# HKUST-Aerial-Robotics/D2SLAM

Measured on AMD Instinct MI355X. Metric: frames/sec SuperPoint+NetVLAD+match, 640x480 stereo, higher is better.
Workload: dtype f32

## Files before the change

d2slam_amd/csrc/conv1x1.hip:

```cpp
#include "conv_common.h"

namespace d2fe {

namespace {
constexpr int C1_CIN = 256, C1_C8 = C1_CIN / 8, C1_RING = 8;
}

__global__ __launch_bounds__(256, 2) void conv1x1_256_65_kernel(ConvArgs a, long npix) {
  extern __shared__ __attribute__((aligned(16))) float wsm[];
  const int tid = threadIdx.x, lane = tid & 63, wave = tid >> 6, hh = lane >> 5;
  const float* wp = reinterpret_cast<const float*>(a.wpack);
  for (int i = tid; i < 2 * C1_C8 * 64; i += 256)
    reinterpret_cast<f32x4*>(wsm)[i] = reinterpret_cast<const f32x4*>(wp)[i];
  float* wdl = wsm + 2 * C1_C8 * 256;
  if (tid < C1_C8 * 8) {
    const int g = tid >> 3, h = (tid >> 2) & 1, q = tid & 3;
    wdl[tid] = wp[((size_t)2 * C1_C8 + g) * 256 + h * 128 + q];
  }
  const float bias0 = a.bias[lane & 31], bias1 = a.bias[32 + (lane & 31)], biasd = a.bias[64];
  __syncthreads();

  const long n_mt = (npix + 31) / 32;
  const int ics = a.in_cstride, ocs = a.out_cstride;
  for (long mt = (long)blockIdx.x * 4 + wave; mt < n_mt; mt += (long)gridDim.x * 4) {
    const long p = mt * 32 + (lane & 31);
    const bool valid = p < npix;
    const float* row = a.in + (size_t)(valid ? p : 0) * ics + a.in_coff;
    f32x16 acc0, acc1;
#pragma unroll
    for (int r = 0; r < 16; ++r) { acc0[r] = bias0; acc1[r] = bias1; }
    float d = biasd;
    f32x4 xa[C1_RING][2];
#pragma unroll
    for (int g = 0; g < C1_RING; ++g) {
      xa[g][0] = *reinterpret_cast<const f32x4*>(row + g * 8);
      xa[g][1] = *reinterpret_cast<const f32x4*>(row + g * 8 + 4);
    }
#pragma unroll 1
    for (int g0 = 0; g0 < C1_C8; g0 += C1_RING) {
#pragma unroll
      for (int gg = 0; gg < C1_RING; ++gg) {
        const int g = g0 + gg;
        const f32x4 x0 = xa[gg][0], x1 = xa[gg][1];
        if (g + C1_RING < C1_C8) {
          xa[gg][0] = *reinterpret_cast<const f32x4*>(row + (g + C1_RING) * 8);
          xa[gg][1] = *reinterpret_cast<const f32x4*>(row + (g + C1_RING) * 8 + 4);
        }
        const f32x4 b0 = reinterpret_cast<const f32x4*>(wsm)[(0 * C1_C8 + g) * 64 + lane];
        const f32x4 b1 = reinterpret_cast<const f32x4*>(wsm)[(1 * C1_C8 + g) * 64 + lane];
        const float a0 = hh ? x0[1] : x0[0], a1 = hh ? x0[3] : x0[2], a2 = hh ? x1[1] : x1[0], a3 = hh ? x1[3] : x1[2];
        acc0 = __builtin_amdgcn_mfma_f32_32x32x2f32(a0, b0[0], acc0, 0, 0, 0);
        acc1 = __builtin_amdgcn_mfma_f32_32x32x2f32(a0, b1[0], acc1, 0, 0, 0);
        acc0 = __builtin_amdgcn_mfma_f32_32x32x2f32(a1, b0[1], acc0, 0, 0, 0);
        acc1 = __builtin_amdgcn_mfma_f32_32x32x2f32(a1, b1[1], acc1, 0, 0, 0);
        acc0 = __builtin_amdgcn_mfma_f32_32x32x2f32(a2, b0[2], acc0, 0, 0, 0);
        acc1 = __builtin_amdgcn_mfma_f32_32x32x2f32(a2, b1[2], acc1, 0, 0, 0);
        acc0 = __builtin_amdgcn_mfma_f32_32x32x2f32(a3, b0[3], acc0, 0, 0, 0);
        acc1 = __builtin_amdgcn_mfma_f32_32x32x2f32(a3, b1[3], acc1, 0, 0, 0);
        const f32x4 we = reinterpret_cast<const f32x4*>(wdl)[g * 2], wo = reinterpret_cast<const f32x4*>(wdl)[g * 2 + 1];
        d = __builtin_fmaf(x0[0], we[0], d);   d = __builtin_fmaf(x0[1], wo[0], d);
        d = __builtin_fmaf(x0[2], we[1], d);   d = __builtin_fmaf(x0[3], wo[1], d);
        d = __builtin_fmaf(x1[0], we[2], d);   d = __builtin_fmaf(x1[1], wo[2], d);
        d = __builtin_fmaf(x1[2], we[3], d);   d = __builtin_fmaf(x1[3], wo[3], d);
      }
    }
    float* out = a.out + a.out_coff;
#pragma unroll
    for (int r = 0; r < 16; ++r) {
      const long pp = mt * 32 + (r & 3) + 8 * (r >> 2) + 4 * hh;
      if (pp < npix) {
        out[(size_t)pp * ocs + (lane & 31)] = acc0[r];
        out[(size_t)pp * ocs + 32 + (lane & 31)] = acc1[r];
      }
    }
    if (valid && hh == 0) out[(size_t)p * ocs + 64] = d;
  }
}

hipError_t launch_conv1x1_256_65(const ConvArgs& a, hipStream_t s) {
  const long hw = (long)a.H * a.W;
  if (a.cout_real != 65 || a.in_img_stride != hw * a.in_cstride || a.out_img_stride != hw * a.out_cstride || a.out_cstride < 65 ||
      (a.in_cstride & 3) || (a.in_coff & 3) || a.in_coff + 256 > a.in_cstride)
    return hipErrorNotSupported;
  const int ncu = a.ncu > 0 ? a.ncu : 256;
  const long npix = hw * a.n_img;
  const long n_wg = (npix + 127) / 128;
  const int grid = (int)(n_wg < 2 * ncu ? n_wg : 2 * ncu);
  constexpr size_t lds = (size_t)(2 * C1_C8 * 256 + C1_C8 * 8) * sizeof(float);
  hipError_t e = hipFuncSetAttribute(reinterpret_cast<const void*>(conv1x1_256_65_kernel), hipFuncAttributeMaxDynamicSharedMemorySize, (int)lds);
  if (e != hipSuccess) return e;
  hipLaunchKernelGGL(conv1x1_256_65_kernel, dim3(grid), dim3(256), lds, s, a, npix);
  return hipGetLastError();
}

}
```

d2slam_amd/csrc/kernels.h:

```cpp
#pragma once
#include <hip/hip_runtime.h>
#include <stdint.h>

#ifdef D2FE_DEVTOOLS
#include <cstdlib>
static inline int d2fe_dev_env(const char* name, int dflt) { const char* e = getenv(name); return e ? atoi(e) : dflt; }
#define D2FE_ABL(a, bits) ((a).ablate & (bits))
#define D2FE_STAMP(buf, wg, i) do { if ((buf) && threadIdx.x == 0) (buf)[(size_t)(wg) * 16 + (i)] = wall_clock64(); } while (0)
#else
static inline int d2fe_dev_env(const char*, int dflt) { return dflt; }
#define D2FE_ABL(a, bits) (0)
#define D2FE_STAMP(buf, wg, i) do {} while (0)
#endif

#ifdef D2FE_DEVTOOLS
#include "../../include/d2fe_debug.h"
namespace d2fe { void regime_note(int regime); void regime_set(int regime, long long value); }
#define D2FE_REGIME(r) ::d2fe::regime_note(r)
#define D2FE_REGIME_SET(r, v) ::d2fe::regime_set(r, v)
#else
#define D2FE_REGIME(r) do {} while (0)
#define D2FE_REGIME_SET(r, v) do {} while (0)
#endif

namespace d2fe {

__host__ __device__ inline bool wino_claims_items(const int* work_ctr, int total, int grid) { return work_ctr != nullptr && total >= 48 * grid; }

struct ConvArgs {
  const float* in;  int in_cstride;  int in_coff;
  float* out;       int out_cstride; int out_coff;
  int cout_real;
  const void* wpack;
  const float* bias;
  int H, W;
  int n_img;
  long in_img_stride;
  long out_img_stride;
  const uint8_t* img; int img_stride; long img_istride; const float* w1a; const float* b1a;
  const float* zeros;
  int tag;
  int ablate;
  int* work_ctr = nullptr;
  int ncu = 0;
};

enum ConvShape {
  CONV_64_T8x32 = 0,
  CONV_128_T4x32,
  CONV_128_T4x16,
  CONV_256_1x1_T4x16,
  CONV1B_FUSED,
};

hipError_t launch_conv(ConvShape shape, int precision, bool pool, bool relu, int cout_pad, const ConvArgs& a,
                       hipStream_t s);

hipError_t launch_conv1x1_256_65(const ConvArgs& a, hipStream_t s);

hipError_t launch_conv_pc(ConvShape shape, int precision, bool pool, bool relu, int cout_pad, const ConvArgs& a, hipStream_t s);

hipError_t launch_conv_wino(int cin, bool pool, bool relu, int cout_pad, const ConvArgs& a, hipStream_t s);
hipError_t launch_conv_wino_fused1b(int cout_pad, const ConvArgs& a, hipStream_t s);
size_t packed_weight_floats_wino(int cout_pad, int cin);
void pack_weights_wino(const float* w , int cout, int cin, int cout_pad, float* dst);

hipError_t launch_conv1a(const uint8_t* img, int stride, long img_stride_bytes, int H, int W, int n,
                         const float* w9x64 , const float* bias, float* out, hipStream_t s);

size_t packed_weight_floats_f32(int cout_pad, int cin, int ks);
void pack_weights_f32(const float* w , int cout, int cin, int ks, int cout_pad, float* dst);
size_t packed_weight_halfs_f16x2(int cout_pad, int cin, int ks);
void pack_weights_f16x2(const float* w, int cout, int cin, int ks, int cout_pad, uint16_t* dst);

hipError_t launch_softmax_cand(const float* logits, int lstride, int Hc, int Wc, int n_img, float thr, int border,
                               float* semi, unsigned long long* cand, int* cand_count, long cand_cap, bool zero_counts, hipStream_t s);
hipError_t launch_select_b(const unsigned long long* cand, const int* cand_count, long cand_cap, int n_img, int W,
                           int max_kp, int cap, int always_sort, const float* semi, int H, float thr, int border, float* kps_xy,
                           float* scores, int32_t* kps_idx, int32_t* n_out, hipStream_t s);
hipError_t launch_sample_b(const float* desc_raw, int dstride, int dcoff, int Hc, int Wc, int n_img, const float* kps_xy,
                           const int32_t* n_kp, int cap, const int32_t* slotmap, int max_slots, float* desc_out, hipStream_t s);
hipError_t launch_desc_head_sparse(const float* kps_xy, const int32_t* n_kp, int cap, int Hc, int Wc, int n_img, const float* x,
                                   int x_cstride, long x_img_stride, const void* w_da, const float* b_da, const void* w_db,
                                   const float* b_db, uint8_t* flags, int32_t* slotmap, int32_t* cells, int32_t* count,
                                   int max_slots, float* out, float* mid, int mid_imgs, int img_w, int img_h, hipStream_t s);

hipError_t launch_nms2_a(const float* semi, int H, int W, int n_img, float thr, int dist, float* aconf, int* clist,
                         unsigned long long* cand, int* cand_count, long cand_cap, int* ncand, hipStream_t s);
hipError_t launch_nms2_wrap_fix(const int* clist, const int* ncand, int H, int W, int n_img, float* kps_xy, int32_t* kps_idx,
                                const int32_t* n_kp, int cap, hipStream_t s);
hipError_t launch_sample_a(const float* desc_raw, int dstride, int dcoff, int Hc, int Wc, int img_w, int img_h, int n_img,
                           const float* kps_xy, const int32_t* n_kp, int cap, const float* comp_t, const float* mean,
                           int pca_dims, float* samp, int scap, float* cn, const int32_t* slotmap, int max_slots, float* desc_out,
                           hipStream_t s);

hipError_t launch_nv_conv0(const uint8_t* img, int stride_b, long img_stride, int H, int W, int Ho, int Wo, int cstride,
                           int cout, int act, const float* w, const float* b, float* out, int n, hipStream_t s);
hipError_t launch_nv_dw(const float* in, int H, int W, int C, int Ho, int Wo, int cstride, int act, const float* w, const float* b,
                        float* out, int n, hipStream_t s);
hipError_t launch_nv_pw(const float* in, long P, int Cin, int Cout, int CoutPad, int act, const float* w, const float* b,
                        const float* res, float* out, hipStream_t s);
hipError_t launch_nv_vlad(const float* x, int slabs, long slab_stride, int np, int D, int K, const float* aw, const float* aw_pack,
                          const float* ab, const float* cen, float* part, float* out, int n, hipStream_t s);
void pack_nv_assign(const float* aw , int K, int D, float* dst);
size_t nv_vlad_part_floats(int np, int D, int K);
hipError_t launch_nv_pca(const float* x, int nfeat, const float* comp, const float* mean, int m, float* y, int n, hipStream_t s);

struct NvBlockArgs {
  const float* in;
  int in_slabs; long in_slab_stride;
  const uint8_t* img; int img_stride; long img_istride; int H0, W0;
  int c0_stride, c0_pt, c0_pl, act0; const float* w0;
  float* out; long out_slab_stride;
  const float* res; int res_slabs; long res_slab_stride;
  int H, W, Cin, Chid, Cout, stride, Ho, Wo, pt, pl;
  int co0, Cv;
  long P;
  int th, tw;
  unsigned inv_iw, inv_tw;
  int cpg;
  int gmerge;
  const float* we;
  const float* wp;
  const float* bp;
  int act_e, act_d, act_p;
  int ncu;
  int tpw;
  int nbuf;
  unsigned long long* stamps;
};
bool nv_block_supported(int cin, int chid, int cout, int stride, bool expand, int mode);
int nv_block_ntiles(int cout);
hipError_t launch_nv_block(const NvBlockArgs& a, bool expand, int mode, int n, int groups, hipStream_t s);
void pack_nv_expand(const float* w , const float* b, int chid, int cin, float* dst);
size_t pack_nv_expand_floats(int chid, int cin);
void pack_nv_dwproj(const float* wd , const float* bd, const float* wp , int cout, int chid, int nt, float* dst);
size_t pack_nv_dwproj_floats(int chid, int nt);
void pack_nv_proj_t(const float* wp, int cout, int chid, int nt, float* dst);
void pack_nv_dwproj_x(const float* wd, const float* bd, const float* wp, int cout, int chid, int nt, float* dst);
void pack_nv_expand_tail(const float* w, const float* b, int chid, int cin, float* dst);
bool nv_tail_supported(int cin, int cout);
hipError_t launch_nv_tail(const NvBlockArgs& a, int groups, hipStream_t s);
bool nv_xblock_supported(int cin, int chid, int cout, int stride);
void nv_xblock_tile(int Ho, int Wo, int stride, int* th, int* tw);
size_t pack_nv_expand_perm_floats(int chid, int cin);
void pack_nv_expand_perm(const float* w, const float* b, int chid, int cin, float* dst);
hipError_t launch_nv_xblock(const NvBlockArgs& a, int n, int groups, hipStream_t s);
bool nv_pblock_supported(int cin, int chid, int cout, int stride);
void nv_pblock_tile(int Ho, int Wo, int* th, int* tw, int c0_stride = 0);
size_t pack_nv_expand_pair_floats(int chid, int cin);
void pack_nv_expand_pair(const float* w, const float* b, int chid, int cin, float* dst);
size_t pack_nv_dwproj_pair_floats(int chid, int nt);
void pack_nv_dwproj_pair(const float* wd, const float* bd, const float* wp, int cout, int chid, int nt, float* dst, int co0 = 0);
int nv_pblock_ntiles(int cout);
int nv_pblock_halves(int cout);
int nv_pblock_half_cout(int cout, int half);
bool nv_pblock_single_input(int cin);
hipError_t launch_nv_pblock(const NvBlockArgs& a, int n, int groups, hipStream_t s);
bool nv_fpair_supported(int c0_cout, int c0_stride, int dw_stride, int cout);
hipError_t launch_nv_fpair(const NvBlockArgs& a, int n, hipStream_t s);
long nv_pblock_slots(int cin, int cout, int ncu, int nbuf);
hipError_t launch_nv_slab_sum(float* t, int slabs, long slab_stride, long count, hipStream_t s, int tree = 1);
bool nv_pblock_can_merge(int cin, int cv);
void pack_nv_conv0(const float* w , const float* b, int cout, float* dst );

hipError_t launch_gen_map(const double* cam9, const double* q4, int mode, int width, int height, double f, float* mapx,
                          float* mapy, hipStream_t s);
hipError_t launch_prep_gray(const uint8_t* src, int ch, int sw, int sh, int sstride, long src_istride, int n, int dw, int dh,
                            uint8_t* dst, hipStream_t s);
hipError_t launch_undistort(const uint8_t* src, int sh, int sw, int sstride, long src_istride, const float* mapx,
                            const float* mapy, const float* gain, int dh, int dw, int n, uint8_t* dst, hipStream_t s);
hipError_t launch_db_search(const float* db, int ntotal, int dim, const float* q, int nq, int k, float* sims_scratch,
                            int32_t* labels, float* out_sims, hipStream_t s);
hipError_t launch_quant_int8(const float* x, int n, int double_max, int8_t* out, hipStream_t s);
hipError_t launch_dequant_int8(const int8_t* q, int n, int landmark_num, float* out, hipStream_t s);

hipError_t launch_pack_blocks(const float* desc, const float* kps, const float* scores, const int32_t* n_kp, const float* gdesc,
                              int row0, int row_step, int nframes, int cap, int G, int blk_words, float* blocks, hipStream_t s);
hipError_t launch_gate_pairs(const float* q, long q_stride, const float* db, long db_stride, int dim, const int32_t* pair_q,
                             const int32_t* pair_db, int npairs, double thres, int32_t* cnt_inout, int32_t* pass, float* sims,
                             int32_t* n_pass, hipStream_t s);
hipError_t launch_pack_blocks_int8(const float* desc, const float* kps, const int32_t* n_kp, const float* gdesc, int row0, int row_step,
                                   int nframes, int cap, int G, int blk_bytes, int8_t* blocks, hipStream_t s);
hipError_t launch_unpack_blocks_int8(const int8_t* blocks, int nblocks, int cap, int G, int blk_bytes, int blk_words, int renorm, float* out,
                                     hipStream_t s);
hipError_t launch_quad_gate(const float* loc, long loc_stride, const float* rem, long rem_stride, int dim, const int32_t* job_loc_row0,
                            const int32_t* job_rem_row0, int loc_view_step, int rem_view_step, int njobs, double thres, int32_t* dir_prev,
                            float* sims, int32_t* cnt_inout, int32_t* n_pass, hipStream_t s);

hipError_t launch_half_compact(const float* desc, const float* pts, const int32_t* n_kp, const int32_t* job_row, const int32_t* job_left,
                               const float* job_shift, int njobs, int cap, int dim, float width_undistort, float move_cols,
                               float* out_desc, float* out_pts, int32_t* out_map, int32_t* out_n, hipStream_t s);
hipError_t launch_half_compact_strided(const float* desc, const float* pts, const int32_t* n_kp, size_t desc_stride, size_t pts_stride, size_t n_stride,
                                       const int32_t* job_row, const int32_t* job_left, const float* job_shift, int njobs, int cap, int dim, float width_undistort,
                                       float move_cols, float* out_desc, float* out_pts, int32_t* out_map, int32_t* out_n, hipStream_t s);
hipError_t launch_remap_matches(int32_t* q_idx, int32_t* t_idx, const int32_t* n_match, const int32_t* map_a_job, const int32_t* map_b_job,
                                const int32_t* maps, int npairs, int cap_match, int cap_map, hipStream_t s);

struct MatchPairDesc { const float* a; const float* b; const float* pts_a; const float* pts_b; const int32_t* na; const int32_t* nb; double radius; };
struct MatchArgs {
  const MatchPairDesc* pairs = nullptr;
  const float* a; const float* b; const float* pts_a; const float* pts_b;
  const int32_t* a_off; const int32_t* b_off; const int32_t* a_cnt; const int32_t* b_cnt;
  int npairs, dim, max_n, mode;
  double ratio, radius;
  int32_t* q_idx; int32_t* t_idx; float* dist; int32_t* n_out;
  int32_t* cand4;
  int32_t* ticket;
  int32_t* stats = nullptr;
  int ncu = 0;
  unsigned long long* stamps = nullptr;
};
hipError_t launch_match(const MatchArgs& m, hipStream_t s);
inline size_t match_scratch_bytes(int npairs, int max_n) { return sizeof(int32_t) * (((size_t)npairs + 15) / 16 * 16 + 8 * (size_t)max_n * npairs); }
inline void match_scratch_carve(void* base, int npairs, MatchArgs* m) { m->ticket = static_cast<int32_t*>(base); m->cand4 = m->ticket + ((size_t)npairs + 15) / 16 * 16; }

}
```

d2slam_amd/csrc/postproc.hip:

```cpp
#include <algorithm>

#include "kernels.h"

namespace d2fe {

typedef float f32x4 __attribute__((ext_vector_type(4)));
typedef float f32x16 __attribute__((ext_vector_type(16)));

__device__ __forceinline__ float d2fe_expf(float x) {
  if (x < -87.0f) x = -87.0f;
  const float t = x * 1.44269504088896341f;
  const float n = __builtin_rintf(t);
  float r = __builtin_fmaf(n, -0.693359375f, x);
  r = __builtin_fmaf(n, 2.12194440e-4f, r);
  float p = 1.9875691500E-4f;
  p = __builtin_fmaf(p, r, 1.3981999507E-3f);
  p = __builtin_fmaf(p, r, 8.3334519073E-3f);
  p = __builtin_fmaf(p, r, 4.1665795894E-2f);
  p = __builtin_fmaf(p, r, 1.6666665459E-1f);
  p = __builtin_fmaf(p, r, 5.0000001201E-1f);
  const float r2 = r * r;
  const float y = __builtin_fmaf(p, r2, r) + 1.0f;
  return __builtin_ldexpf(y, (int)n);
}
// ... 305 lines not shown
  const int k = blockIdx.x * 4 + (threadIdx.x >> 6);
  if (k >= n_kp[img] || k >= cap) return;
  const size_t o = (size_t)img * cap + k;
  const SampleBCorners c = sample_b_corners(kps_xy[2 * o], kps_xy[2 * o + 1], Hc, Wc);
  f32x4 v[4];
  float nrm[4];
#pragma unroll
  for (int q = 0; q < 4; ++q) {
    const int cell = c.iy[q] * Wc + c.ix[q];
    const float* row = slotmap ? desc_raw + ((size_t)img * max_slots + slotmap[(size_t)img * Hc * Wc + cell]) * 256
                               : desc_raw + ((size_t)img * Hc * Wc + cell) * dstride + dcoff;
    v[q] = *reinterpret_cast<const f32x4*>(row + lane * 4);
    nrm[q] = __builtin_sqrtf(wave_sum(v[q][0] * v[q][0] + v[q][1] * v[q][1] + v[q][2] * v[q][2] + v[q][3] * v[q][3]));
  }
  f32x4 d;
  float ss = 0.f;
#pragma unroll
  for (int j = 0; j < 4; ++j) {
    float t = (v[0][j] / nrm[0]) * c.w[0];
    t = t + (v[1][j] / nrm[1]) * c.w[1];
    t = t + (v[2][j] / nrm[2]) * c.w[2];
    t = t + (v[3][j] / nrm[3]) * c.w[3];
    d[j] = t;
    ss += t * t;
  }
  ss = wave_sum(ss);
  const float ninv = (float)(1.0 / (double)__builtin_sqrtf(ss));
#pragma unroll
  for (int j = 0; j < 4; ++j) d[j] = d[j] * ninv;
  *reinterpret_cast<f32x4*>(desc_out + o * 256 + lane * 4) = d;
}

__device__ __forceinline__ void sample_a_origin(float x, float y, int Hc, int Wc, int img_w, int img_h, float& ix, float& iy) {
  const float gx = 2.0f * x / (float)img_w - 1.0f;
  const float gy = 2.0f * y / (float)img_h - 1.0f;
  ix = ((gx + 1.0f) * (float)Wc - 1.0f) / 2.0f;
  iy = ((gy + 1.0f) * (float)Hc - 1.0f) / 2.0f;
}

__global__ __launch_bounds__(256) void desc_mark_kernel(const float* __restrict__ kps_xy, const int32_t* __restrict__ n_kp, int cap,
                                                        int Hc, int Wc, int img_w, int img_h, uint8_t* __restrict__ flags) {
  const int img = blockIdx.y, k = blockIdx.x * 256 + threadIdx.x;
  if (k >= n_kp[img] || k >= cap) return;
  const size_t o = (size_t)img * cap + k;
  uint8_t* f = flags + (size_t)img * Hc * Wc;
  if (img_w > 0) {
    float ix, iy;
    sample_a_origin(kps_xy[2 * o], kps_xy[2 * o + 1], Hc, Wc, img_w, img_h, ix, iy);
    const int x0 = (int)__builtin_floorf(ix), y0 = (int)__builtin_floorf(iy);
#pragma unroll
    for (int q = 0; q < 4; ++q) {
      const int xx = x0 + (q & 1), yy = y0 + (q >> 1);
      if (yy >= 0 && yy < Hc && xx >= 0 && xx < Wc) f[yy * Wc + xx] = 1;
    }
    return;
  }
  const SampleBCorners c = sample_b_corners(kps_xy[2 * o], kps_xy[2 * o + 1], Hc, Wc);
#pragma unroll
  for (int q = 0; q < 4; ++q) f[c.iy[q] * Wc + c.ix[q]] = 1;
}

__global__ __launch_bounds__(1024) void desc_compact_kernel(const uint8_t* __restrict__ flags, int ncell, int max_slots,
                                                            int32_t* __restrict__ slotmap, int32_t* __restrict__ cells,
                                                            int32_t* __restrict__ count) {
  __shared__ int wsum[16];
  __shared__ int s_base;
  const int img = blockIdx.x, tid = threadIdx.x, lane = tid & 63, wv = tid >> 6;
  if (tid == 0) s_base = 0;
  __syncthreads();
  for (int c0 = 0; c0 < ncell; c0 += 1024) {
    const int cell = c0 + tid;
    const bool f = cell < ncell && flags[(size_t)img * ncell + cell];
    const unsigned long long bal = __ballot(f);
    if (lane == 0) wsum[wv] = __popcll(bal);
    __syncthreads();
    int pre = 0, tot = 0;
#pragma unroll
    for (int k = 0; k < 16; ++k) { const int c = wsum[k]; pre += k < wv ? c : 0; tot += c; }
    const int slot = s_base + pre + __popcll(bal & ((1ull << lane) - 1ull));
    if (cell < ncell) slotmap[(size_t)img * ncell + cell] = (f && slot < max_slots) ? slot : -1;
    if (f && slot < max_slots) cells[(size_t)img * max_slots + slot] = cell;
    __syncthreads();
    if (tid == 0) s_base += tot;
    __syncthreads();
  }
  if (tid == 0) count[img] = s_base < max_slots ? s_base : max_slots;
}

__global__ __launch_bounds__(1024) void desc_mark_compact_kernel(const float* __restrict__ kps_xy, const int32_t* __restrict__ n_kp, int cap, int Hc, int Wc,
                                                                 int img_w, int img_h, int max_slots, int32_t* __restrict__ slotmap,
                                                                 int32_t* __restrict__ cells, int32_t* __restrict__ count) {
  extern __shared__ uint8_t mc_flags[];
  __shared__ int wsum[16];
  __shared__ int s_base;
  const int img = blockIdx.x, tid = threadIdx.x, lane = tid & 63, wv = tid >> 6;
  const int ncell = Hc * Wc;
  for (int i = tid; i < (ncell + 3) / 4; i += 1024) reinterpret_cast<uint32_t*>(mc_flags)[i] = 0u;
  if (tid == 0) s_base = 0;
  __syncthreads();
  const int nk = min(n_kp[img], cap);
  for (int k = tid; k < nk; k += 1024) {
    const size_t o = (size_t)img * cap + k;
    if (img_w > 0) {
      float ix, iy;
      sample_a_origin(kps_xy[2 * o], kps_xy[2 * o + 1], Hc, Wc, img_w, img_h, ix, iy);
      const int x0 = (int)__builtin_floorf(ix), y0 = (int)__builtin_floorf(iy);
#pragma unroll
      for (int q = 0; q < 4; ++q) {
        const int xx = x0 + (q & 1), yy = y0 + (q >> 1);
        if (yy >= 0 && yy < Hc && xx >= 0 && xx < Wc) mc_flags[yy * Wc + xx] = 1;
      }
    } else {
      const SampleBCorners c = sample_b_corners(kps_xy[2 * o], kps_xy[2 * o + 1], Hc, Wc);
#pragma unroll
      for (int q = 0; q < 4; ++q) mc_flags[c.iy[q] * Wc + c.ix[q]] = 1;
    }
  }
  __syncthreads();
  for (int c0 = 0; c0 < ncell; c0 += 1024) {
    const int cell = c0 + tid;
    const bool f = cell < ncell && mc_flags[cell];
    const unsigned long long bal = __ballot(f);
    if (lane == 0) wsum[wv] = __popcll(bal);
    __syncthreads();
    int pre = 0, tot = 0;
#pragma unroll
    for (int k = 0; k < 16; ++k) { const int c = wsum[k]; pre += k < wv ? c : 0; tot += c; }
    const int slot = s_base + pre + __popcll(bal & ((1ull << lane) - 1ull));
    if (cell < ncell) slotmap[(size_t)img * ncell + cell] = (f && slot < max_slots) ? slot : -1;
    if (f && slot < max_slots) cells[(size_t)img * max_slots + slot] = cell;
    __syncthreads();
    if (tid == 0) s_base += tot;
    __syncthreads();
  }
  if (tid == 0) count[img] = s_base < max_slots ? s_base : max_slots;
}

struct SparseHeadArgs {
  const float* x; int x_cstride; long x_img_stride;
  const void* w_da; const float* b_da;
  const void* w_db; const float* b_db;
  const int32_t* cells; const int32_t* count; int max_slots;
  int Hc, Wc;
  float* out;
  float* mid;
};

template <int MT, int NW, int STAGE>
__global__ __launch_bounds__(64 * NW) void desc_head_sparse_kernel(SparseHeadArgs a) {
  constexpr int CIN = 128, CPA = CIN + 1, CMID = 256, CPD = CMID + 1, G = 4, M = 32 * MT, NT = 64 * NW;
  static_assert((NW == 8 && STAGE == 0) || (NW == 4 && STAGE != 0 && MT == 1), "whole head: 8 waves x 32 channels; split stages: 4 waves per channel half");
  extern __shared__ __attribute__((aligned(16))) float sparse_lds[];
  float* A = sparse_lds;
  float* D = sparse_lds;
  int* s_cell = reinterpret_cast<int*>(sparse_lds + M * CPD);
  const int img = blockIdx.y, mt = blockIdx.x;
  const int n = a.count[img];
  if (mt * M >= n) return;
  const int tid = threadIdx.x, lane = tid & 63, wave = tid >> 6;
  if (tid < M) s_cell[tid] = mt * M + tid < n ? a.cells[(size_t)img * a.max_slots + mt * M + tid] : -1;
  __syncthreads();
  const float* x = a.x + (size_t)img * a.x_img_stride;
  const f32x4* wda = reinterpret_cast<const f32x4*>(a.w_da);
  const f32x4* wdb = reinterpret_cast<const f32x4*>(a.w_db);
  const int nt0 = (STAGE == 0 ? 0 : (int)blockIdx.z * NW) + wave;
  float* mid = a.mid + ((size_t)img * a.max_slots + mt * M) * 256;

  f32x16 acc[MT];
  if constexpr (STAGE != 2) {
    {
      const float b = a.b_da[nt0 * 32 + (lane & 31)];
#pragma unroll
      for (int m = 0; m < MT; ++m)
#pragma unroll
        for (int r = 0; r < 16; ++r) acc[m][r] = b;
    }
    const int arow = (lane & 31) * CPA + (lane >> 5);
    constexpr int NG = M * (CIN / 4) / NT;
    for (int tap = 0; tap < 9; ++tap) {
      __syncthreads();
      f32x4 gv[NG];
#pragma unroll
      for (int j = 0; j < NG; ++j) {
        const int i = tid + NT * j;
        const int row = i / (CIN / 4), c4 = i % (CIN / 4);
        const int cell = s_cell[row];
        const int cy = cell / a.Wc + tap / 3 - 1, cx = cell % a.Wc + tap % 3 - 1;
        const bool ok = cell >= 0 && cy >= 0 && cy < a.Hc && cx >= 0 && cx < a.Wc;
        const f32x4 v = *reinterpret_cast<const f32x4*>(x + (ok ? ((size_t)cy * a.Wc + cx) * a.x_cstride + c4 * 4 : 0));
        gv[j] = ok ? v : f32x4{0.f, 0.f, 0.f, 0.f};
      }
#pragma unroll
      for (int j = 0; j < NG; ++j) {
        const int i = tid + NT * j;
        const int row = i / (CIN / 4), c4 = i % (CIN / 4);
        float* d = A + row * CPA + c4 * 4;
        d[0] = gv[j][0]; d[1] = gv[j][1]; d[2] = gv[j][2]; d[3] = gv[j][3];
      }
      __syncthreads();
#pragma unroll 1
      for (int g = 0; g < (CIN / 8) / G; ++g) {
        f32x4 bq[G];
#pragma unroll
        for (int j = 0; j < G; ++j) bq[j] = wda[((size_t)(nt0 * 9 + tap) * (CIN / 8) + g * G + j) * 64 + lane];
#pragma unroll
        for (int j = 0; j < G; ++j) {
          const float* ap = A + arow + (g * G + j) * 8;
#pragma unroll
          for (int q = 0; q < 4; ++q)
#pragma unroll
            for (int m = 0; m < MT; ++m) acc[m] = __builtin_amdgcn_mfma_f32_32x32x2f32(ap[m * 32 * CPA + 2 * q], bq[j][q], acc[m], 0, 0, 0);
        }
      }
    }
    if constexpr (STAGE == 1) {
#pragma unroll
      for (int r = 0; r < 16; ++r) {
        const int row = (r & 3) + 8 * (r >> 2) + 4 * (lane >> 5);
        const float v = acc[0][r];
        if (mt * M + row < n) mid[(size_t)row * 256 + nt0 * 32 + (lane & 31)] = v > 0.f ? v : 0.f;
      }
      return;
    }
    __syncthreads();
#pragma unroll
    for (int m = 0; m < MT; ++m)
#pragma unroll
      for (int r = 0; r < 16; ++r) {
        const int row = m * 32 + (r & 3) + 8 * (r >> 2) + 4 * (lane >> 5);
        const float v = acc[m][r];
        D[row * CPD + nt0 * 32 + (lane & 31)] = v > 0.f ? v : 0.f;
      }
    __syncthreads();
  } else {
    constexpr int ND = M * (CMID / 4) / NT;
    f32x4 dv[ND];
#pragma unroll
    for (int j = 0; j < ND; ++j) {
      const int i = tid + NT * j;
      const int row = i / (CMID / 4), c4 = i % (CMID / 4);
      dv[j] = mt * M + row < n ? *reinterpret_cast<const f32x4*>(mid + (size_t)row * 256 + c4 * 4) : f32x4{0.f, 0.f, 0.f, 0.f};
    }
#pragma unroll
    for (int j = 0; j < ND; ++j) {
      const int i = tid + NT * j;
      const int row = i / (CMID / 4), c4 = i % (CMID / 4);
      float* d = D + row * CPD + c4 * 4;
      d[0] = dv[j][0]; d[1] = dv[j][1]; d[2] = dv[j][2]; d[3] = dv[j][3];
    }
    __syncthreads();
  }
  {
    const float b = a.b_db[nt0 * 32 + (lane & 31)];
#pragma unroll
    for (int m = 0; m < MT; ++m)
#pragma unroll
      for (int r = 0; r < 16; ++r) acc[m][r] = b;
  }
  const int drow = (lane & 31) * CPD + (lane >> 5);
#pragma unroll 1
  for (int g = 0; g < (CMID / 8) / G; ++g) {
    f32x4 bq[G];
#pragma unroll
    for (int j = 0; j < G; ++j) bq[j] = wdb[((size_t)nt0 * (CMID / 8) + g * G + j) * 64 + lane];
#pragma unroll
    for (int j = 0; j < G; ++j) {
      const float* ap = D + drow + (g * G + j) * 8;
#pragma unroll
      for (int q = 0; q < 4; ++q)
#pragma unroll
        for (int m = 0; m < MT; ++m) acc[m] = __builtin_amdgcn_mfma_f32_32x32x2f32(ap[m * 32 * CPD + 2 * q], bq[j][q], acc[m], 0, 0, 0);
    }
  }
  float* out = a.out + ((size_t)img * a.max_slots + mt * M) * 256;
#pragma unroll
  for (int m = 0; m < MT; ++m)
#pragma unroll
    for (int r = 0; r < 16; ++r) {
      const int row = m * 32 + (r & 3) + 8 * (r >> 2) + 4 * (lane >> 5);
      if (mt * M + row < n) out[(size_t)row * 256 + nt0 * 32 + (lane & 31)] = acc[m][r];
    }
}

hipError_t launch_desc_head_sparse(const float* kps_xy, const int32_t* n_kp, int cap, int Hc, int Wc, int n_img, const float* x,
                                   int x_cstride, long x_img_stride, const void* w_da, const float* b_da, const void* w_db,
                                   const float* b_db, uint8_t* flags, int32_t* slotmap, int32_t* cells, int32_t* count,
                                   int max_slots, float* out, float* mid, int mid_imgs, int img_w, int img_h, hipStream_t s) {
  const int ncell = Hc * Wc;
  hipError_t e = hipSuccess;
  if (ncell <= 60 * 1024) {
    hipLaunchKernelGGL(desc_mark_compact_kernel, dim3(n_img), dim3(1024), (size_t)(ncell + 3) / 4 * 4, s, kps_xy, n_kp, cap, Hc, Wc, img_w, img_h, max_slots, slotmap, cells, count);
  } else {
    e = hipMemsetAsync(flags, 0, (size_t)n_img * ncell, s);
    if (e != hipSuccess) return e;
    hipLaunchKernelGGL(desc_mark_kernel, dim3((cap + 255) / 256, n_img), dim3(256), 0, s, kps_xy, n_kp, cap, Hc, Wc, img_w, img_h, flags);
    hipLaunchKernelGGL(desc_compact_kernel, dim3(n_img), dim3(1024), 0, s, flags, ncell, max_slots, slotmap, cells, count);
  }
  SparseHeadArgs a;
  a.x = x; a.x_cstride = x_cstride; a.x_img_stride = x_img_stride; a.w_da = w_da; a.b_da = b_da; a.w_db = w_db; a.b_db = b_db;
  a.cells = cells; a.count = count; a.max_slots = max_slots; a.Hc = Hc; a.Wc = Wc; a.out = out; a.mid = mid;
  const int slots = std::min(max_slots, 4 * cap);
  if (n_img >= 8) {
    constexpr size_t lds = sizeof(float) * (64 * 257 + 64);
    e = hipFuncSetAttribute(reinterpret_cast<const void*>(desc_head_sparse_kernel<2, 8, 0>), hipFuncAttributeMaxDynamicSharedMemorySize, (int)lds);
    if (e != hipSuccess) return e;
    hipLaunchKernelGGL((desc_head_sparse_kernel<2, 8, 0>), dim3((slots + 63) / 64, n_img), dim3(512), lds, s, a);
  } else if (mid && n_img <= mid_imgs && n_img <= 4) {
    const dim3 grid((slots + 31) / 32, n_img, 2);
    hipLaunchKernelGGL((desc_head_sparse_kernel<1, 4, 1>), grid, dim3(256), sizeof(float) * (32 * 257 + 32), s, a);
    hipLaunchKernelGGL((desc_head_sparse_kernel<1, 4, 2>), grid, dim3(256), sizeof(float) * (32 * 257 + 32), s, a);
  } else {
    hipLaunchKernelGGL((desc_head_sparse_kernel<1, 8, 0>), dim3((slots + 31) / 32, n_img), dim3(512), sizeof(float) * (32 * 257 + 32), s, a);
  }
  return hipGetLastError();
}

hipError_t launch_sample_b(const float* desc_raw, int dstride, int dcoff, int Hc, int Wc, int n_img, const float* kps_xy,
                           const int32_t* n_kp, int cap, const int32_t* slotmap, int max_slots, float* desc_out, hipStream_t s) {
  dim3 grid((cap + 3) / 4, n_img), block(256);
  hipLaunchKernelGGL(sample_b_kernel, grid, block, 0, s, desc_raw, dstride, dcoff, Hc, Wc, kps_xy, n_kp, cap, slotmap, max_slots,
                     desc_out);
  return hipGetLastError();
}

__global__ __launch_bounds__(1024) void nms2_a_kernel(const float* __restrict__ semi, int H, int W, float thr, int d,
                                                      float* __restrict__ aconf, int* __restrict__ clist,
                                                      unsigned long long* __restrict__ cand, int* __restrict__ cand_count,
                                                      long cand_cap, int* __restrict__ iters_out,
                                                      int* __restrict__ ncand_out) {
  __shared__ int s_n, s_changed;
  const int img = blockIdx.x, tid = threadIdx.x;
  const size_t hw = (size_t)H * W;
  const float* sm = semi + img * hw;
  float* ac = aconf + img * hw;
  int* cl = clist + img * hw;
  __shared__ int s_wcnt[16];
  const int lane = tid & 63, wv = tid >> 6;
  const size_t seg = ((hw + 15) / 16 + 63) / 64 * 64;
  const size_t seg0 = wv * seg, seg1 = (seg0 + seg < hw) ? seg0 + seg : hw;
  int wcnt = 0;
  for (size_t i0 = seg0; i0 < seg1; i0 += 64) {
    const size_t i = i0 + lane;
    const float p = i < seg1 ? sm[i] : 0.f;
    const bool c = i < seg1 && p > thr;
    if (i < seg1) ac[i] = c ? p : 0.f;
    wcnt += __popcll(__ballot(c));
  }
  if (lane == 0) s_wcnt[wv] = wcnt;
  __syncthreads();
  int wbase = 0, n = 0;
  for (int w = 0; w < 16; ++w) { if (w < wv) wbase += s_wcnt[w]; n += s_wcnt[w]; }
  for (size_t i0 = seg0; i0 < seg1; i0 += 64) {
    const size_t i = i0 + lane;
    const bool c = i < seg1 && sm[i] > thr;
    const unsigned long long m = __ballot(c);
    if (c) cl[wbase + __popcll(m & ((1ull << lane) - 1ull))] = (int)i;
    wbase += __popcll(m);
  }
  if (tid == 0) { s_n = n; if (ncand_out) ncand_out[img] = n; }
  __syncthreads();
  int iters = 0;
  for (;;) {
    if (tid == 0) s_changed = 0;
    __syncthreads();
    for (int k = tid; k < n; k += 1024) {
      const int i = cl[k];
      const int x = i % W, y = i / W;
      const float p = sm[i];
      bool sup = false;
      for (int yy = max(0, y - d); yy <= y; ++yy) {
        const int x1 = (yy == y) ? x - 1 : min(W - 1, x + d);
        for (int xx = max(0, x - d); xx <= x1; ++xx) sup |= (ac[(size_t)yy * W + xx] > p);
      }
      const float want = sup ? 0.f : p;
      if (ac[i] != want) { ac[i] = want; s_changed = 1; }
    }
    __syncthreads();
    ++iters;
    const int ch = s_changed;
    __syncthreads();
    if (!ch) break;
  }
  if (tid == 0 && iters_out) iters_out[img] = iters;
  unsigned long long* cd = cand + (size_t)img * cand_cap;
  for (int k = tid; k < n; k += 1024) {
    const int i = cl[k];
    const float p = sm[i];
    if (ac[i] == 0.f) continue;
    const int x = i % W, y = i / W;
    bool dead = false;
    for (int yy = y; yy <= min(H - 1, y + d); ++yy) {
      const int x0 = (yy == y) ? x + 1 : max(0, x - d);
      for (int xx = x0; xx <= min(W - 1, x + d); ++xx) dead |= (ac[(size_t)yy * W + xx] > p);
    }
    if (!dead) {
      const int slot = atomicAdd(cand_count + img, 1);
      if (slot < cand_cap) cd[slot] = ((unsigned long long)__float_as_uint(p) << 32) | (unsigned long long)(0xFFFFFFFFu - (unsigned)i);
    }
  }
}

hipError_t launch_nms2_a(const float* semi, int H, int W, int n_img, float thr, int dist, float* aconf, int* clist,
                         unsigned long long* cand, int* cand_count, long cand_cap, int* ncand, hipStream_t s) {
  hipError_t e = hipMemsetAsync(cand_count, 0, sizeof(int) * n_img, s);
  if (e != hipSuccess) return e;
  hipLaunchKernelGGL(nms2_a_kernel, dim3(n_img), dim3(1024), 0, s, semi, H, W, thr, dist, aconf, clist, cand, cand_count,
                     cand_cap, (int*)nullptr, ncand);
  return hipGetLastError();
}

__global__ __launch_bounds__(256) void nms2_wrap_fix_kernel(const int* __restrict__ clist, const int* __restrict__ ncand, int H, int W,
                                                            float* __restrict__ kps_xy, int32_t* __restrict__ kps_idx,
                                                            const int32_t* __restrict__ n_kp, int cap) {
  const int img = blockIdx.y;
  const int n = ncand[img];
  if (n <= 65536) return;
  const int k = blockIdx.x * 256 + threadIdx.x;
  if (k >= n_kp[img] || k >= cap) return;
  const int* cl = clist + (size_t)img * H * W;
  float* kp = kps_xy + ((size_t)img * cap + k) * 2;
  const int i = (int)kp[1] * W + (int)kp[0];
  int lo = 0, hi = n;
  while (lo < hi) { const int mid = (lo + hi) >> 1; if (cl[mid] < i) lo = mid + 1; else hi = mid; }
  const int j = cl[lo & 0xFFFF];
  kp[0] = (float)(j % W); kp[1] = (float)(j / W);
  if (kps_idx) kps_idx[(size_t)img * cap + k] = j;
}
hipError_t launch_nms2_wrap_fix(const int* clist, const int* ncand, int H, int W, int n_img, float* kps_xy, int32_t* kps_idx,
                                const int32_t* n_kp, int cap, hipStream_t s) {
  hipLaunchKernelGGL(nms2_wrap_fix_kernel, dim3((cap + 255) / 256, n_img), dim3(256), 0, s, clist, ncand, H, W, kps_xy, kps_idx, n_kp, cap);
  return hipGetLastError();
}

__global__ __launch_bounds__(256) void sample_a_kernel(const float* __restrict__ desc_raw, int dstride, int dcoff, int Hc,
                                                       int Wc, int img_w, int img_h, const float* __restrict__ kps_xy,
                                                       const int32_t* __restrict__ n_kp, int cap, int scap,
                                                       const int32_t* __restrict__ slotmap, int max_slots,
                                                       float* __restrict__ samp) {
  const int img = blockIdx.y;
  const int lane = threadIdx.x & 63, wv = threadIdx.x >> 6;
  const int k = blockIdx.x * 4 + wv;
  if (k >= n_kp[img] || k >= cap || k >= scap) return;
  const size_t o = (size_t)img * cap + k;
  float ix, iy;
  sample_a_origin(kps_xy[2 * o], kps_xy[2 * o + 1], Hc, Wc, img_w, img_h, ix, iy);
  const int x0 = (int)__builtin_floorf(ix), y0 = (int)__builtin_floorf(iy), x1 = x0 + 1, y1 = y0 + 1;
  const float nw = ((float)x1 - ix) * ((float)y1 - iy);
  const float ne = (ix - (float)x0) * ((float)y1 - iy);
  const float sw = ((float)x1 - ix) * (iy - (float)y0);
  const float se = (ix - (float)x0) * (iy - (float)y0);
  const float* base = desc_raw + (size_t)img * Hc * Wc * dstride + dcoff + lane * 4;
  auto corner = [&](int yy, int xx, float wgt, f32x4& acc) {
    if (yy < 0 || yy >= Hc || xx < 0 || xx >= Wc) return;
    const float* row = slotmap ? desc_raw + ((size_t)img * max_slots + slotmap[(size_t)img * Hc * Wc + yy * Wc + xx]) * 256 + lane * 4
                               : base + ((size_t)yy * Wc + xx) * dstride;
    const f32x4 v = *reinterpret_cast<const f32x4*>(row);
    const float nrm = __builtin_sqrtf(wave_sum(v[0] * v[0] + v[1] * v[1] + v[2] * v[2] + v[3] * v[3]));
#pragma unroll
    for (int j = 0; j < 4; ++j) acc[j] = acc[j] + (v[j] / nrm) * wgt;
  };
  f32x4 d = {0.f, 0.f, 0.f, 0.f};
  corner(y0, x0, nw, d); corner(y0, x1, ne, d); corner(y1, x0, sw, d); corner(y1, x1, se, d);
  *reinterpret_cast<f32x4*>(samp + ((size_t)img * scap + k) * 256 + lane * 4) = d;
}

__global__ __launch_bounds__(256) void chan_norm_a_kernel(const float* __restrict__ samp, const int32_t* __restrict__ n_kp, int cap,
                                                          int scap, float* __restrict__ cn) {
  const int img = blockIdx.x, c = threadIdx.x;
  const int n = min(min(n_kp[img], cap), scap);
  const float* s = samp + (size_t)img * scap * 256 + c;
  float ss = 0.f;
  for (int k = 0; k < n; ++k) { const float v = s[(size_t)k * 256]; ss += v * v; }
  cn[img * 256 + c] = __builtin_sqrtf(ss);
}

__global__ __launch_bounds__(256) void finish_a_kernel(const float* __restrict__ samp, const float* __restrict__ cn,
                                                       const int32_t* __restrict__ n_kp, int cap, int scap,
                                                       const float* __restrict__ comp_t, const float* __restrict__ mean,
                                                       int pca_dims, float* __restrict__ desc_out) {
  __shared__ float sd[4][256];
  const int img = blockIdx.y;
  const int lane = threadIdx.x & 63, wv = threadIdx.x >> 6;
  const int k = blockIdx.x * 4 + wv;
  if (k >= n_kp[img] || k >= cap || k >= scap) return;
  const size_t o = (size_t)img * cap + k;
  f32x4 d = *reinterpret_cast<const f32x4*>(samp + ((size_t)img * scap + k) * 256 + lane * 4);
  const f32x4 c4 = *reinterpret_cast<const f32x4*>(cn + img * 256 + lane * 4);
#pragma unroll
  for (int j = 0; j < 4; ++j) d[j] = d[j] / c4[j];
  if (!comp_t) {
    const float ss = wave_sum(d[0] * d[0] + d[1] * d[1] + d[2] * d[2] + d[3] * d[3]);
    const float n2 = __builtin_sqrtf(ss);
#pragma unroll
    for (int j = 0; j < 4; ++j) d[j] = d[j] / n2;
    *reinterpret_cast<f32x4*>(desc_out + o * 256 + lane * 4) = d;
    return;
  }
#pragma unroll
  for (int j = 0; j < 4; ++j) sd[wv][lane * 4 + j] = d[j] - mean[lane * 4 + j];
  __builtin_amdgcn_wave_barrier();
  for (int j0 = 0; j0 < pca_dims; j0 += 64) {
    const int j = j0 + lane;
    float a = 0.f;
    if (j < pca_dims)
      for (int c = 0; c < 256; ++c) a += sd[wv][c] * comp_t[(size_t)c * pca_dims + j];
    float s2 = wave_sum(j < pca_dims ? a * a : 0.f);
    if (pca_dims <= 64) {
      const float n2 = __builtin_sqrtf(s2);
      if (j < pca_dims) desc_out[o * pca_dims + j] = a / n2;
    } else {
      if (j < pca_dims) desc_out[o * pca_dims + j] = a;
    }
  }
  if (pca_dims > 64) {
    __builtin_amdgcn_wave_barrier();
    float s2 = 0.f;
    for (int j = lane; j < pca_dims; j += 64) { const float a = desc_out[o * pca_dims + j]; s2 += a * a; }
    s2 = wave_sum(s2);
    const float n2 = __builtin_sqrtf(s2);
    for (int j = lane; j < pca_dims; j += 64) desc_out[o * pca_dims + j] = desc_out[o * pca_dims + j] / n2;
  }
}

hipError_t launch_sample_a(const float* desc_raw, int dstride, int dcoff, int Hc, int Wc, int img_w, int img_h, int n_img,
                           const float* kps_xy, const int32_t* n_kp, int cap, const float* comp_t, const float* mean,
                           int pca_dims, float* samp, int scap, float* cn, const int32_t* slotmap, int max_slots, float* desc_out,
                           hipStream_t s) {
  const int kmax = cap < scap ? cap : scap;
  dim3 grid((kmax + 3) / 4, n_img), block(256);
  hipLaunchKernelGGL(sample_a_kernel, grid, block, 0, s, desc_raw, dstride, dcoff, Hc, Wc, img_w, img_h, kps_xy, n_kp, cap, scap, slotmap,
                     max_slots, samp);
  hipLaunchKernelGGL(chan_norm_a_kernel, dim3(n_img), block, 0, s, samp, n_kp, cap, scap, cn);
  hipLaunchKernelGGL(finish_a_kernel, grid, block, 0, s, samp, cn, n_kp, cap, scap, comp_t, mean, pca_dims, desc_out);
  return hipGetLastError();
}

}
```

Before: 2361.

## Stage conv1x1 input through swizzled LDS with double-buffered cross-tile prefetch

The 1x1 conv (256->65) kernel now has 8 waves per block, one block per CU. Each wave loads its 32-pixel tile cooperatively in coalesced 64-channel pieces into a per-wave XOR-swizzled LDS area, and prefetches the next tile's pieces into registers during compute. Operands are software-pipelined with sched barriers. hipFuncSetAttribute calls are cached per device to cut host overhead on every launch. This uses more LDS and fewer blocks, and per-lane strided global reads are replaced by LDS round-trips.

```diff
diff --git a/d2slam_amd/csrc/conv1x1.hip b/d2slam_amd/csrc/conv1x1.hip
--- a/d2slam_amd/csrc/conv1x1.hip
+++ b/d2slam_amd/csrc/conv1x1.hip
@@ -1,16 +1,30 @@
+#include <atomic>
+
 #include "conv_common.h"
 
 namespace d2fe {
 
 namespace {
-constexpr int C1_CIN = 256, C1_C8 = C1_CIN / 8, C1_RING = 8;
+constexpr int C1_CIN = 256, C1_C8 = C1_CIN / 8, C1_NW = 8;
+constexpr int C1_PC = 64, C1_NPC = C1_CIN / C1_PC, C1_PV = 32 * C1_PC / 4 / 64;
+constexpr int C1_WFLOATS = 2 * C1_C8 * 256 + C1_C8 * 8;
+static_assert(C1_PC == 64 && C1_NPC % 2 == 0, "the swizzle is written for 16 slots per pixel row; two register sets alternate");
+
+__device__ __forceinline__ void c1_request(f32x4 (&v)[C1_PV], const float* piece, int lr, int ls, int nvalid, int ics) {
+#pragma unroll
+  for (int j = 0; j < C1_PV; ++j) {
+    const int r = j * 4 + lr;
+    const unsigned off = (unsigned)((r < nvalid ? r : nvalid - 1) * ics + ls * 4) * 4u;
+    v[j] = *reinterpret_cast<const f32x4*>(reinterpret_cast<const char*>(piece) + off);
+  }
+}
 }
 
-__global__ __launch_bounds__(256, 2) void conv1x1_256_65_kernel(ConvArgs a, long npix) {
+__global__ __launch_bounds__(64 * C1_NW) void conv1x1_256_65_kernel(ConvArgs a, long npix) {
   extern __shared__ __attribute__((aligned(16))) float wsm[];
-  const int tid = threadIdx.x, lane = tid & 63, wave = tid >> 6, hh = lane >> 5;
+  const int tid = threadIdx.x, lane = tid & 63, wave = __builtin_amdgcn_readfirstlane(tid >> 6), hh = lane >> 5;
   const float* wp = reinterpret_cast<const float*>(a.wpack);
-  for (int i = tid; i < 2 * C1_C8 * 64; i += 256)
+  for (int i = tid; i < 2 * C1_C8 * 64; i += 64 * C1_NW)
     reinterpret_cast<f32x4*>(wsm)[i] = reinterpret_cast<const f32x4*>(wp)[i];
   float* wdl = wsm + 2 * C1_C8 * 256;
   if (tid < C1_C8 * 8) {
@@ -20,34 +34,62 @@
   const float bias0 = a.bias[lane & 31], bias1 = a.bias[32 + (lane & 31)], biasd = a.bias[64];
   __syncthreads();
 
-  const long n_mt = (npix + 31) / 32;
+  const long n_mt = (npix + 31) / 32, step = (long)gridDim.x * C1_NW;
+  long mt = blockIdx.x + (long)gridDim.x * wave;
+  if (mt >= n_mt) return;
   const int ics = a.in_cstride, ocs = a.out_cstride;
-  for (long mt = (long)blockIdx.x * 4 + wave; mt < n_mt; mt += (long)gridDim.x * 4) {
-    const long p = mt * 32 + (lane & 31);
-    const bool valid = p < npix;
-    const float* row = a.in + (size_t)(valid ? p : 0) * ics + a.in_coff;
+  const int lr = lane >> 4, ls = lane & 15, px = lane & 31;
+  const float* in0 = a.in + a.in_coff;
+  float* aw = wsm + C1_WFLOATS + wave * (32 * C1_PC);
+  const float* ar = aw + px * C1_PC;
+  const int pxs = px & 15;
+  f32x4 st[2][C1_PV];
+  {
+    const float* tb = in0 + (size_t)mt * 32 * ics;
+    const int nv = (int)(npix - mt * 32 < 32 ? npix - mt * 32 : 32);
+    c1_request(st[0], tb, lr, ls, nv, ics);
+    c1_request(st[1], tb + C1_PC, lr, ls, nv, ics);
+  }
+#pragma unroll 1
+  for (; mt < n_mt; mt += step) {
+    const long nx = mt + step;
+    const bool more = nx < n_mt;
+    const float* tb = in0 + (size_t)mt * 32 * ics;
+    const float* nb = in0 + (size_t)(more ? nx : mt) * 32 * ics;
+    const int nv = (int)(npix - mt * 32 < 32 ? npix - mt * 32 : 32), nnv = (int)(more && npix - nx * 32 < 32 ? npix - nx * 32 : 32);
     f32x16 acc0, acc1;
 #pragma unroll
     for (int r = 0; r < 16; ++r) { acc0[r] = bias0; acc1[r] = bias1; }
     float d = biasd;
-    f32x4 xa[C1_RING][2];
+#pragma unroll 1
+    for (int pc2 = 0; pc2 < C1_NPC; pc2 += 2) {
 #pragma unroll
-    for (int g = 0; g < C1_RING; ++g) {
-      xa[g][0] = *reinterpret_cast<const f32x4*>(row + g * 8);
-      xa[g][1] = *reinterpret_cast<const f32x4*>(row + g * 8 + 4);
-    }
-#pragma unroll 1
-    for (int g0 = 0; g0 < C1_C8; g0 += C1_RING) {
+    for (int pi = 0; pi < 2; ++pi) {
+      const int pc = pc2 + pi;
+      int bo = lane * 4, dwo = 2 * C1_C8 * 256;
+      asm volatile("" : "+v"(bo), "+v"(dwo));
+      const f32x4* bw = reinterpret_cast<const f32x4*>(wsm + bo);
+      const f32x4* dw = reinterpret_cast<const f32x4*>(wsm + dwo);
 #pragma unroll
-      for (int gg = 0; gg < C1_RING; ++gg) {
-        const int g = g0 + gg;
-        const f32x4 x0 = xa[gg][0], x1 = xa[gg][1];
-        if (g + C1_RING < C1_C8) {
-          xa[gg][0] = *reinterpret_cast<const f32x4*>(row + (g + C1_RING) * 8);
-          xa[gg][1] = *reinterpret_cast<const f32x4*>(row + (g + C1_RING) * 8 + 4);
-        }
-        const f32x4 b0 = reinterpret_cast<const f32x4*>(wsm)[(0 * C1_C8 + g) * 64 + lane];
-        const f32x4 b1 = reinterpret_cast<const f32x4*>(wsm)[(1 * C1_C8 + g) * 64 + lane];
+      for (int j = 0; j < C1_PV; ++j) {
+        const int r = j * 4 + lr;
+        *reinterpret_cast<f32x4*>(aw + r * C1_PC + ((ls ^ (r & 15)) * 4)) = st[pi][j];
+      }
+      if (pc2 == 0 || more) c1_request(st[pi], (pc2 == 0 ? tb + 2 * C1_PC : nb) + pi * C1_PC, lr, ls, pc2 == 0 ? nv : nnv, ics);
+      f32x4 ox[2][2], ob[2][2], od[2][2];
+      auto operands = [&](int gg, int set) {
+        const int g = pc * (C1_PC / 8) + gg;
+        ox[set][0] = *reinterpret_cast<const f32x4*>(ar + (((2 * gg) ^ pxs) * 4));
+        ox[set][1] = *reinterpret_cast<const f32x4*>(ar + (((2 * gg + 1) ^ pxs) * 4));
+        ob[set][0] = bw[(0 * C1_C8 + g) * 64]; ob[set][1] = bw[(1 * C1_C8 + g) * 64];
+        od[set][0] = dw[g * 2]; od[set][1] = dw[g * 2 + 1];
+      };
+      operands(0, 0);
+#pragma unroll
+      for (int gg = 0; gg < C1_PC / 8; ++gg) {
+        if (gg + 1 < C1_PC / 8) operands(gg + 1, (gg + 1) & 1);
+        __builtin_amdgcn_sched_barrier(0);
+        const f32x4 x0 = ox[gg & 1][0], x1 = ox[gg & 1][1], b0 = ob[gg & 1][0], b1 = ob[gg & 1][1], we = od[gg & 1][0], wo = od[gg & 1][1];
         const float a0 = hh ? x0[1] : x0[0], a1 = hh ? x0[3] : x0[2], a2 = hh ? x1[1] : x1[0], a3 = hh ? x1[3] : x1[2];
         acc0 = __builtin_amdgcn_mfma_f32_32x32x2f32(a0, b0[0], acc0, 0, 0, 0);
         acc1 = __builtin_amdgcn_mfma_f32_32x32x2f32(a0, b1[0], acc1, 0, 0, 0);
@@ -57,23 +99,26 @@
         acc1 = __builtin_amdgcn_mfma_f32_32x32x2f32(a2, b1[2], acc1, 0, 0, 0);
         acc0 = __builtin_amdgcn_mfma_f32_32x32x2f32(a3, b0[3], acc0, 0, 0, 0);
         acc1 = __builtin_amdgcn_mfma_f32_32x32x2f32(a3, b1[3], acc1, 0, 0, 0);
-        const f32x4 we = reinterpret_cast<const f32x4*>(wdl)[g * 2], wo = reinterpret_cast<const f32x4*>(wdl)[g * 2 + 1];
         d = __builtin_fmaf(x0[0], we[0], d);   d = __builtin_fmaf(x0[1], wo[0], d);
         d = __builtin_fmaf(x0[2], we[1], d);   d = __builtin_fmaf(x0[3], wo[1], d);
         d = __builtin_fmaf(x1[0], we[2], d);   d = __builtin_fmaf(x1[1], wo[2], d);
         d = __builtin_fmaf(x1[2], we[3], d);   d = __builtin_fmaf(x1[3], wo[3], d);
+        asm volatile("" : "+v"(d));
+        __builtin_amdgcn_sched_barrier(0);
       }
+    }
     }
     float* out = a.out + a.out_coff;
 #pragma unroll
     for (int r = 0; r < 16; ++r) {
       const long pp = mt * 32 + (r & 3) + 8 * (r >> 2) + 4 * hh;
       if (pp < npix) {
-        out[(size_t)pp * ocs + (lane & 31)] = acc0[r];
-        out[(size_t)pp * ocs + 32 + (lane & 31)] = acc1[r];
+        out[(size_t)pp * ocs + px] = acc0[r];
+        out[(size_t)pp * ocs + 32 + px] = acc1[r];
       }
     }
-    if (valid && hh == 0) out[(size_t)p * ocs + 64] = d;
+    const long p = mt * 32 + px;
+    if (p < npix && hh == 0) out[(size_t)p * ocs + 64] = d;
   }
 }
 
@@ -84,12 +129,14 @@
     return hipErrorNotSupported;
   const int ncu = a.ncu > 0 ? a.ncu : 256;
   const long npix = hw * a.n_img;
-  const long n_wg = (npix + 127) / 128;
-  const int grid = (int)(n_wg < 2 * ncu ? n_wg : 2 * ncu);
-  constexpr size_t lds = (size_t)(2 * C1_C8 * 256 + C1_C8 * 8) * sizeof(float);
-  hipError_t e = hipFuncSetAttribute(reinterpret_cast<const void*>(conv1x1_256_65_kernel), hipFuncAttributeMaxDynamicSharedMemorySize, (int)lds);
+  if (npix <= 0) return hipSuccess;
+  const long n_mt = (npix + 31) / 32;
+  const int grid = (int)(n_mt < ncu ? n_mt : ncu);
+  constexpr size_t lds = (size_t)(C1_WFLOATS + C1_NW * 32 * C1_PC) * sizeof(float);
+  static std::atomic<unsigned long long> lds_set{0};
+  hipError_t e = max_dyn_lds_once(reinterpret_cast<const void*>(conv1x1_256_65_kernel), (int)lds, lds_set);
   if (e != hipSuccess) return e;
-  hipLaunchKernelGGL(conv1x1_256_65_kernel, dim3(grid), dim3(256), lds, s, a, npix);
+  hipLaunchKernelGGL(conv1x1_256_65_kernel, dim3(grid), dim3(64 * C1_NW), lds, s, a, npix);
   return hipGetLastError();
 }
 
diff --git a/d2slam_amd/csrc/kernels.h b/d2slam_amd/csrc/kernels.h
--- a/d2slam_amd/csrc/kernels.h
+++ b/d2slam_amd/csrc/kernels.h
@@ -1,6 +1,8 @@
 #pragma once
 #include <hip/hip_runtime.h>
 #include <stdint.h>
+
+#include <atomic>
 
 #ifdef D2FE_DEVTOOLS
 #include <cstdlib>
@@ -26,6 +28,17 @@
 namespace d2fe {
 
 __host__ __device__ inline bool wino_claims_items(const int* work_ctr, int total, int grid) { return work_ctr != nullptr && total >= 48 * grid; }
+
+inline hipError_t max_dyn_lds_once(const void* kernel, int bytes, std::atomic<unsigned long long>& done) {
+  int dev = 0;
+  hipError_t e = hipGetDevice(&dev);
+  if (e != hipSuccess) return e;
+  const unsigned long long bit = dev >= 0 && dev < 64 ? 1ull << dev : 0ull;
+  if (bit && (done.load(std::memory_order_acquire) & bit)) return hipSuccess;
+  e = hipFuncSetAttribute(kernel, hipFuncAttributeMaxDynamicSharedMemorySize, bytes);
+  if (e == hipSuccess && bit) done.fetch_or(bit, std::memory_order_release);
+  return e;
+}
 
 struct ConvArgs {
   const float* in;  int in_cstride;  int in_coff;
diff --git a/d2slam_amd/csrc/postproc.hip b/d2slam_amd/csrc/postproc.hip
--- a/d2slam_amd/csrc/postproc.hip
+++ b/d2slam_amd/csrc/postproc.hip
@@ -631,7 +631,8 @@
   const int slots = std::min(max_slots, 4 * cap);
   if (n_img >= 8) {
     constexpr size_t lds = sizeof(float) * (64 * 257 + 64);
-    e = hipFuncSetAttribute(reinterpret_cast<const void*>(desc_head_sparse_kernel<2, 8, 0>), hipFuncAttributeMaxDynamicSharedMemorySize, (int)lds);
+    static std::atomic<unsigned long long> lds_set{0};
+    e = max_dyn_lds_once(reinterpret_cast<const void*>(desc_head_sparse_kernel<2, 8, 0>), (int)lds, lds_set);
     if (e != hipSuccess) return e;
     hipLaunchKernelGGL((desc_head_sparse_kernel<2, 8, 0>), dim3((slots + 63) / 64, n_img), dim3(512), lds, s, a);
   } else if (mid && n_img <= mid_imgs && n_img <= 4) {
```

Result: no change. 2347 (-0.6%).
